# mills-lab/vapor

Hardware: AMD Instinct MI355X
Metric: SV loci validated/sec (higher is better)
Workload: dtype u32

## Files before the change

### vapor_amd/csrc/vapor_hip.hip

```cpp
#include "vapor_kernels.h"
#include "vapor_wide.h"
#include "vapor_anyk.h"
#include "vapor_realign.h"
#include "vapor_realign_trace.h"
#include "vapor_bamdev.h"
#include "vapor_bgzf.h"
#include "vapor_fasta.h"
#include "vapor_refine.h"
#include "vapor_planner.h"
#include "vapor_readplan.h"
#include "vapor_hip.h"

#include <unistd.h>

#include <algorithm>
#include <cstdio>
#include <cstdlib>
#include <cstring>
#include <new>
#include <numeric>
#include <map>
#include <memory>
#include <mutex>
#include <set>
// ... 23 lines not shown

struct BlockPool {
    std::multimap<size_t, void*> free_dev, free_host;
    std::map<const void*, size_t> cap_of;
    size_t cached_dev = 0, cached_host = 0;
};
static std::mutex g_live_m;
static std::set<const void*> g_live_ctx;

static size_t pool_round(size_t bytes)
{
    if (bytes <= 256) return 256;
    if (bytes < ((size_t)1 << 16)) { size_t c = 256; while (c < bytes) c <<= 1; return c; }
    return (bytes + 0xFFFF) & ~(size_t)0xFFFF;
}

struct vapor_ctx {
    int device = 0;
    hipStream_t stream = nullptr;
    hipStream_t own_stream = nullptr;
    hipStream_t lane[2] = {nullptr, nullptr};
    hipStream_t fin[2] = {nullptr, nullptr};
    unsigned lane_rr = 0;
    bool user_stream = false;
    uint8_t* h_stage = nullptr;
    uint8_t* d_stage = nullptr;
    size_t stage_cap = 0;
    std::vector<double> h_gt;
    double* d_gt = nullptr;
    int reads_per_task = MAX_READS_PER_TASK;
    int n_cus = 256;
    int join_tasks = 256;
    int64_t max_pair_cap = (int64_t)1 << 28;
    bool shared_join = true;
    int remap_in_clean = 1;
    int clean_order = 1;
    int clean_fit = 1;
    int64_t trace_budget = vapor_trace::BUDGET_DEFAULT;
    int stage_threads = 3;
    bool attrs_set = false;
    uint32_t* d_crc_pow = nullptr;
    std::map<const uint8_t*, size_t> arenas;
    hipStream_t bam_stream = nullptr;
    int bam_stream_share = 0;
    int bam_cu_share = 0;
    hipEvent_t bam_ev[2] = {nullptr, nullptr};
    double bam_stats[7] = {0, 0, 0, 0, 0, 0, 0};
    hipEvent_t fasta_ev[2] = {nullptr, nullptr};
    double fasta_stats[6] = {0, 0, 0, 0, 0, 0};
    BlockPool pool;
};

static bool ctx_alive(const vapor_ctx* c)
{
    std::lock_guard<std::mutex> g(g_live_m);
// ... 97 lines not shown
    int32_t n_lit = 0;
    std::vector<SeqDesc> h;
    SeqDesc* d_seqs = nullptr;
    uint32_t *d_p2 = nullptr, *d_e1 = nullptr, *d_x4 = nullptr;
    size_t plane_chunks = 0;
    std::vector<std::vector<HSeg>> derived;
    std::vector<ShareGroup> groups;
    std::vector<int32_t> group_of, slot_of;
    uint8_t* d_raw = nullptr;
    std::vector<int64_t> raw_off;
};

struct vapor_plan : PlanLayout {
    vapor_ctx* ctx = nullptr;
    int device = 0;
    vapor_seqset* set = nullptr;
    int64_t n_pairs = 0;
    std::vector<int64_t> last_stats;
    int hcap_want = 4096;
    bool hcap_measured = false;
    int64_t total_cap = 0;
    DPair* d_pairs = nullptr;
    DTask* d_tasks = nullptr;
    int32_t* d_task_pairs = nullptr;
    unsigned long long* d_hits = nullptr;
    uint8_t* d_hflags = nullptr;
    unsigned long long* d_nhits = nullptr;
    long long* d_stats = nullptr;
    long long* h_stats = nullptr;
    hipEvent_t ev[4] = {nullptr, nullptr, nullptr, nullptr};
    hipEvent_t ev_f[2] = {nullptr, nullptr};
    std::vector<std::array<hipEvent_t, 4>> ring;
    int ring_n = 0;
    bool overflow_final = false;
    double acc_ms[4] = {0, 0, 0, 0};
    int64_t acc_n = 0;
    double* h_loci = nullptr;
    hipEvent_t ev_t0 = nullptr;
    hipStream_t lane = nullptr;
    hipStream_t fin = nullptr;
    hipEvent_t ev_clean = nullptr;
    hipEvent_t ev_fin = nullptr;
    bool have_fin = false;
    hipEvent_t ev_last = nullptr;
    hipEvent_t ev_after = nullptr;
    bool have_last = false, have_after = false;
    double t_join = 0, t_clean = 0, t_total = 0;
    int n_retried = 0;
    bool ran = false;
    bool flags_valid = false;
    int64_t n_reads = 0, n_loci = 0;
    DRead* d_reads = nullptr;
    int32_t* d_locus_first = nullptr;
    double* d_gt = nullptr;
    bool own_gt = false;
    double* d_read_scores = nullptr;
    double* d_loci = nullptr;
    unsigned int* d_overflow = nullptr;
    int32_t* d_big_list = nullptr;
    unsigned int* h_overflow = nullptr;
    bool big_known = false;
    unsigned int n_big = 0;
// ... 99 lines not shown
        if (e) (void)hipEventDestroy(e);
    for (hipEvent_t e : c->fasta_ev)
        if (e) (void)hipEventDestroy(e);
    delete c;
    return VAPOR_OK;
}

extern "C" int vapor_set_param(vapor_ctx* c, const char* name, int64_t v)
{
    if (!c || !name) return fail(VAPOR_E_ARG, "vapor_set_param: null argument");
    if (!strcmp(name, "reads_per_task")) {
        if (v < 1 || v > MAX_READS_PER_TASK) return fail(VAPOR_E_ARG, "reads_per_task out of range");
        c->reads_per_task = (int)v;
        return VAPOR_OK;
    }
    if (!strcmp(name, "bam_cu_share")) {
        if (v < 0 || v > 8) return fail(VAPOR_E_ARG, "bam_cu_share out of range (0 .. 8 eighths of the CUs; 0 and 8: all)");
        c->bam_cu_share = (int)(v == 8 ? 0 : v);
        return VAPOR_OK;
    }
    if (!strcmp(name, "join_tasks")) {
        if (v < 1) return fail(VAPOR_E_ARG, "join_tasks out of range");
        c->join_tasks = (int)v;
        return VAPOR_OK;
    }
    if (!strcmp(name, "max_pair_cap")) {
        if (v < 1) return fail(VAPOR_E_ARG, "max_pair_cap out of range");
        c->max_pair_cap = v;
        return VAPOR_OK;
    }
    if (!strcmp(name, "shared_join")) {
        c->shared_join = v != 0;
        return VAPOR_OK;
    }
    if (!strcmp(name, "remap_in_clean")) {
        if (v < 0 || v > 2) return fail(VAPOR_E_ARG, "vapor_set_param: remap_in_clean is 0, 1 or 2");
        c->remap_in_clean = (int)v;
        return VAPOR_OK;
    }
    if (!strcmp(name, "clean_order")) {
        c->clean_order = v != 0 ? 1 : 0;
        return VAPOR_OK;
    }
    if (!strcmp(name, "clean_fit")) {
        c->clean_fit = v != 0;
        return VAPOR_OK;
// ... 845 lines not shown

static void plan_free_grid(vapor_plan* p)
{
    dfree(p->ctx, p->d_grid); p->d_grid = nullptr;
    dfree(p->ctx, p->d_group_out); p->d_group_out = nullptr;
    dfree(p->ctx, p->d_winner_scores); p->d_winner_scores = nullptr;
    p->n_groups = 0;
}

static void plan_free_reads(vapor_plan* p)
{
    dfree(p->ctx, p->d_reads); p->d_reads = nullptr;
    p->d_locus_first = nullptr;
    if (p->own_gt) dfree(p->ctx, p->d_gt);
    p->d_gt = nullptr; p->own_gt = false;
    dfree(p->ctx, p->d_read_scores); p->d_read_scores = nullptr;
    dfree(p->ctx, p->d_loci); p->d_loci = nullptr;
}

static void plan_free_device(vapor_plan* p)
{
    dfree(p->ctx, p->d_pairs); p->d_pairs = nullptr;
    dfree(p->ctx, p->d_tasks); p->d_tasks = nullptr;
    dfree(p->ctx, p->d_task_pairs); p->d_task_pairs = nullptr;
    dfree(p->ctx, p->d_hits); p->d_hits = nullptr;
    dfree(p->ctx, p->d_hflags); p->d_hflags = nullptr;
    dfree(p->ctx, p->d_nhits); p->d_nhits = nullptr;
    dfree(p->ctx, p->d_stats); p->d_stats = nullptr;
    plan_free_reads(p);
    dfree(p->ctx, p->d_shares); p->d_shares = nullptr;
    dfree(p->ctx, p->d_maps); p->d_maps = nullptr;
    dfree(p->ctx, p->d_serve); p->d_serve = nullptr;
    dfree(p->ctx, p->d_clean_order); p->d_clean_order = nullptr;
    plan_free_grid(p);
}

extern "C" int vapor_plan_destroy(vapor_plan* p)
{
    if (!p) return VAPOR_OK;
    (void)hipSetDevice(p->device);
    if (p->ring_n > 0 && p->lane && ctx_alive(p->ctx)) {
        (void)hipStreamSynchronize(p->lane);
        if (p->fin) (void)hipStreamSynchronize(p->fin);
    }
    plan_free_device(p);
    hfree(p->ctx, p->h_stats);
    hfree(p->ctx, p->h_overflow);
    dfree(p->ctx, p->d_overflow);
    dfree(p->ctx, p->d_big_list);
    for (auto& e : p->ev)
        if (e) (void)hipEventDestroy(e);
    for (auto& r : p->ring)
        for (auto& e : r)
            if (e) (void)hipEventDestroy(e);
    hfree(p->ctx, p->h_loci);
    for (auto& e : p->ev_f)
        if (e) (void)hipEventDestroy(e);
    if (p->ev_t0) (void)hipEventDestroy(p->ev_t0);
    if (p->ev_last) (void)hipEventDestroy(p->ev_last);
    if (p->ev_clean) (void)hipEventDestroy(p->ev_clean);
    if (p->ev_fin) (void)hipEventDestroy(p->ev_fin);
    if (p->ev_after) (void)hipEventDestroy(p->ev_after);
    delete p;
    return VAPOR_OK;
}

static_assert((2 * VAPOR_MAX_SEQ_LEN + 2 + 31) / 32 <= CLEAN_RANGE_WORDS_MAX, "cluster_axis sizes its per-thread word list for this");
// ... 15 lines not shown
    HIPCHK(hipMemcpyAsync(p->d_pairs, p->hp.data(), sizeof(DPair) * p->hp.size(), hipMemcpyHostToDevice, p->ctx->stream));
    if (p->n_dpairs) {
        for (auto& sv : p->serve)
            if (sv.dpair >= 0) { sv.hit_off = p->hp[(size_t)sv.dpair].hit_off; sv.cap = p->hp[(size_t)sv.dpair].cap; }
        HIPCHK(hipMemcpyAsync(p->d_serve, p->serve.data(), sizeof(DServe) * p->serve.size(), hipMemcpyHostToDevice, p->ctx->stream));
    }
    return VAPOR_OK;
}

extern "C" int vapor_plan_create(vapor_ctx* ctx, vapor_seqset* set, int64_t n_pairs, const vapor_pair* pairs,
                                 vapor_plan** out)
{
    if (!ctx || !set || !out || n_pairs < 0 || (n_pairs && !pairs))
        return fail(VAPOR_E_ARG, "vapor_plan_create: null argument");
    if (n_pairs > 0x7FFFFFF0LL) return fail(VAPOR_E_ARG, "too many pairs");
    HIPCHK(hipSetDevice(ctx->device));
    CallScope sc(ctx, ctx->stream);
    std::unique_ptr<vapor_plan, Building<vapor_plan, vapor_plan_destroy>> p(new (std::nothrow) vapor_plan(), {&sc});
    if (!p) return fail(VAPOR_E_NOMEM, "out of memory");
    p->ctx = ctx;
    p->device = ctx->device;
    p->set = set;
    p->n_pairs = n_pairs;
    static_cast<PlanLayout&>(*p) = plan_layout(PlanParams{ctx->reads_per_task, ctx->join_tasks, ctx->max_pair_cap, ctx->shared_join,
                                                          tile_pos<JoinCfg, 2>(), tile_pos<JoinCfg, 4>()},
                                               SetView{set->h, set->n, set->n_lit, set->derived, set->groups, set->group_of, set->slot_of},
                                               n_pairs, pairs);
    p->hcap_want = (int)std::min<int64_t>(p->hwant, CLEAN_HCAP_MAX);
    p->n_dpairs = (int64_t)p->shares.size();
    HIPCHK(dmalloc(ctx, (void**)&p->d_pairs, sizeof(DPair) * p->hp.size()));
    HIPCHK(dmalloc(ctx, (void**)&p->d_tasks, sizeof(DTask) * std::max<size_t>(p->tasks.size(), 1)));
    HIPCHK(dmalloc(ctx, (void**)&p->d_task_pairs, sizeof(int32_t) * std::max<size_t>(p->task_pairs.size(), 1)));
    HIPCHK(dmalloc(ctx, (void**)&p->d_nhits, sizeof(unsigned long long) * p->hp.size()));
    HIPCHK(hipMemsetAsync(p->d_nhits, 0, sizeof(unsigned long long) * p->hp.size(), ctx->stream));
    HIPCHK(dmalloc(ctx, (void**)&p->d_stats, sizeof(long long) * 16 * p->hp.size()));
    HIPCHK(hmalloc(ctx, (void**)&p->h_stats, sizeof(long long) * 16 * p->hp.size()));
    HIPCHK(dmalloc(ctx, (void**)&p->d_overflow, 4 * sizeof(unsigned int)));
    HIPCHK(hipMemsetAsync(p->d_overflow, 0, 4 * sizeof(unsigned int), ctx->stream));
    HIPCHK(dmalloc(ctx, (void**)&p->d_big_list, sizeof(int32_t) * p->hp.size()));
    HIPCHK(hmalloc(ctx, (void**)&p->h_overflow, 2 * sizeof(unsigned int)));
    if (p->n_dpairs) {
        HIPCHK(dmalloc(ctx, (void**)&p->d_shares, sizeof(DShare) * p->shares.size()));
        HIPCHK(dmalloc(ctx, (void**)&p->d_maps, sizeof(int32_t) * std::max<size_t>(p->tables.size(), 1)));
        HIPCHK(dmalloc(ctx, (void**)&p->d_serve, sizeof(DServe) * p->serve.size()));
        HIPCHK(hipMemcpyAsync(p->d_shares, p->shares.data(), sizeof(DShare) * p->shares.size(), hipMemcpyHostToDevice, ctx->stream));
        if (!p->tables.empty())
            HIPCHK(hipMemcpyAsync(p->d_maps, p->tables.data(), sizeof(int32_t) * p->tables.size(), hipMemcpyHostToDevice, ctx->stream));
    }
    if (ctx->clean_order && n_pairs > 1 && n_pairs <= (int64_t)8 * (2048 / CLEAN_THREADS) * ctx->n_cus) {
        HIPCHK(dmalloc(ctx, (void**)&p->d_clean_order, sizeof(int32_t) * (size_t)n_pairs));
        const std::vector<int32_t> ord = clean_order(*p, n_pairs);
        HIPCHK(hipMemcpy(p->d_clean_order, ord.data(), sizeof(int32_t) * (size_t)n_pairs, hipMemcpyHostToDevice));
    }
    for (auto& e : p->ev) HIPCHK(hipEventCreate(&e));
    for (auto& e : p->ev_f) HIPCHK(hipEventCreate(&e));
    HIPCHK(hipEventCreate(&p->ev_t0));
    if (!p->tasks.empty())
        HIPCHK(hipMemcpyAsync(p->d_tasks, p->tasks.data(), sizeof(DTask) * p->tasks.size(), hipMemcpyHostToDevice, ctx->stream));
    if (!p->task_pairs.empty())
        HIPCHK(hipMemcpyAsync(p->d_task_pairs, p->task_pairs.data(), sizeof(int32_t) * p->task_pairs.size(), hipMemcpyHostToDevice, ctx->stream));
    if (const int rc = plan_alloc_hits(p.get())) return rc;
    HIPCHK(hipStreamSynchronize(ctx->stream));
    p->last_stats.assign((size_t)n_pairs * 16, 0);
    *out = p.release();
    return VAPOR_OK;
}

template <int BPS, int K>
static void launch_join(vapor_plan* p, const Launch& L, bool first, hipStream_t st)
{
    const vapor_seqset* s = p->set;
    if (BPS == 2 && L.exc == 1)
        hipLaunchKernelGGL((join_kernel<JoinCfg, BPS, K, (BPS == 2 ? 1 : 0)>), dim3((unsigned)L.n_tasks), dim3(JoinCfg::THREADS), JOIN_DYN_LDS(BPS),
                           st, s->d_seqs, s->d_p2, s->d_e1, s->d_x4, p->d_pairs, p->d_tasks + L.task_begin,
                           p->d_task_pairs, p->d_hits, p->d_nhits, first ? p->d_overflow : (unsigned int*)nullptr);
    else if (BPS == 2 && L.exc == 2)
        hipLaunchKernelGGL((join_kernel<JoinCfg, BPS, K, (BPS == 2 ? 2 : 0)>), dim3((unsigned)L.n_tasks), dim3(JoinCfg::THREADS), JOIN_DYN_LDS(BPS),
                           st, s->d_seqs, s->d_p2, s->d_e1, s->d_x4, p->d_pairs, p->d_tasks + L.task_begin,
                           p->d_task_pairs, p->d_hits, p->d_nhits, first ? p->d_overflow : (unsigned int*)nullptr);
    else
        hipLaunchKernelGGL((join_kernel<JoinCfg, BPS, K, 0>), dim3((unsigned)L.n_tasks), dim3(JoinCfg::THREADS), JOIN_DYN_LDS(BPS),
                           st, s->d_seqs, s->d_p2, s->d_e1, s->d_x4, p->d_pairs, p->d_tasks + L.task_begin,
                           p->d_task_pairs, p->d_hits, p->d_nhits, first ? p->d_overflow : (unsigned int*)nullptr);
}

static int clean_groups_cap(int range_words_cap) { return range_words_cap * 32 / 10 + 8; }

template <typename... A>
static void launch_clean(int range_words_cap, unsigned grid, size_t lds, hipStream_t st, A... a)
{
    const int per = (range_words_cap + CLEAN_THREADS - 1) / CLEAN_THREADS;
    if (per <= 4) hipLaunchKernelGGL(clean_kernel<4>, dim3(grid), dim3(CLEAN_THREADS), lds, st, a...);
    else if (per <= 8) hipLaunchKernelGGL(clean_kernel<8>, dim3(grid), dim3(CLEAN_THREADS), lds, st, a...);
    else hipLaunchKernelGGL(clean_kernel<CLEAN_PER_MAX>, dim3(grid), dim3(CLEAN_THREADS), lds, st, a...);
}

constexpr int CLEAN_BIG_GRID = 1024;

static size_t clean_fixed_bytes(int rw, bool wide)
{
    const size_t g = (size_t)clean_groups_cap(rw);
    return sizeof(uint32_t) * ((size_t)rw + ((size_t)rw + 1) / 2 + (wide ? g : (g + 1) / 2)) + 64;
}

static int clean_groups_lds(int rw, int hcap)
// ... 23 lines not shown
        if (cap >= (exact ? want : want * 9 / 10) || per_cu == 1) { g.hcap = std::max(cap, 0); g.per_cu = per_cu; break; }
    }
    return g;
}
static CleanGeom clean_geom(int range_words_cap, int want, bool exact = false)
{
    const CleanGeom seq = clean_geom_for(range_words_cap, want, false, exact), dual = clean_geom_for(range_words_cap, want, true, exact);
#ifdef VAPOR_DEV_BUILD
    if (const char* e = getenv("VAPOR_DEV_CLEAN_DUAL")) return atoi(e) ? dual : seq;
#endif
    return dual.per_cu >= seq.per_cu ? dual : seq;
}

static int async_fold(vapor_plan* p);

static bool remap_in_clean(const vapor_plan* p)
{
    if (p->n_dpairs <= 0 || p->ctx->remap_in_clean == 0) return false;
    if (p->ctx->remap_in_clean == 2) return true;
    const CleanGeom cg = clean_geom(p->range_words_cap, p->hcap_want, p->hcap_measured);
    return p->n_pairs <= 4 * (int64_t)cg.per_cu * p->ctx->n_cus;
}

static int plan_run_once(vapor_plan* p, bool fetch_stats = true, hipEvent_t* evs = nullptr, hipStream_t on = nullptr, bool skip_big = false,
                         hipEvent_t before_clean = nullptr, bool keep_flags = true)
{
    vapor_ctx* c = p->ctx;
    hipStream_t st = on ? on : c->stream;
    hipEvent_t* ev = evs ? evs : p->ev;
    if (p->launches.empty()) HIPCHK(hipMemsetAsync(p->d_overflow, 0, 2 * sizeof(unsigned int), st));
    HIPCHK(hipEventRecord(ev[0], st));
    bool first = true;
    for (const Launch& L : p->launches) {
        if (L.bps == 2) {
            if (L.k == 10) launch_join<2, 10>(p, L, first, st);
            else if (L.k == 20) launch_join<2, 20>(p, L, first, st);
            else if (L.k == 30) launch_join<2, 30>(p, L, first, st);
            else launch_join<2, 40>(p, L, first, st);
        } else {
            if (L.k == 10) launch_join<4, 10>(p, L, first, st);
            else if (L.k == 20) launch_join<4, 20>(p, L, first, st);
            else if (L.k == 30) launch_join<4, 30>(p, L, first, st);
            else launch_join<4, 40>(p, L, first, st);
        }
        first = false;
        HIPCHK(hipGetLastError());
    }
#if defined(VAPOR_AB) && VAPOR_AB == 3
    if (false) {
#else
    if (p->n_dpairs && !remap_in_clean(p)) {
#endif
        hipLaunchKernelGGL(remap_kernel, dim3((unsigned)p->n_dpairs), dim3(256), 0, st, (const DPair*)p->d_pairs, (const DShare*)p->d_shares,
                           (const int32_t*)p->d_maps, p->d_hits, p->d_nhits, p->d_overflow);
        HIPCHK(hipGetLastError());
    }
    HIPCHK(hipEventRecord(ev[1], st));
    if (before_clean) HIPCHK(hipStreamWaitEvent(st, before_clean, 0));
    if (p->n_pairs > 0) {
        const CleanGeom cg = clean_geom(p->range_words_cap, p->hcap_want, p->hcap_measured);
        const int hcap = cg.hcap;
        size_t lds = clean_lds_bytes(p->range_words_cap, hcap, cg.dual);
#ifdef VAPOR_DEV_BUILD
        if (const char* e = getenv("VAPOR_DEV_CLEAN_PAD")) lds += (size_t)atoi(e);
#endif
        const bool in_clean = remap_in_clean(p);
// ... 15 lines not shown
    if (p->n_pairs > 0 && fetch_stats)
        HIPCHK(hipMemcpyAsync(p->h_stats, p->d_stats, sizeof(long long) * 16 * (size_t)p->n_pairs, hipMemcpyDeviceToHost, st));
    if (!fetch_stats) return VAPOR_OK;
    HIPCHK(hipEventRecord(ev[3], st));
    HIPCHK(hipStreamSynchronize(st));
    float a = 0, b = 0, t = 0;
    HIPCHK(hipEventElapsedTime(&a, ev[0], ev[1]));
    HIPCHK(hipEventElapsedTime(&b, ev[1], ev[2]));
    HIPCHK(hipEventElapsedTime(&t, ev[0], ev[3]));
    p->t_join = a; p->t_clean = b; p->t_total = t;
    return VAPOR_OK;
}

extern "C" int vapor_plan_run(vapor_plan* p, int64_t* stats)
{
    if (!p || (p->n_pairs && !stats)) return fail(VAPOR_E_ARG, "vapor_plan_run: null argument");
    HIPCHK(hipSetDevice(p->ctx->device));
    if (p->ring_n > 0) {
        int rc0 = async_fold(p);
        if (rc0 != VAPOR_OK) return rc0;
    }
    p->n_retried = 0;
    for (int attempt = 0; attempt < 3; ++attempt) {
        int rc = plan_run_once(p);
        if (rc != VAPOR_OK) return rc;
        int64_t grow = 0;
        for (int64_t i = 0; i < p->n_pairs; ++i) {
            const long long* s = p->h_stats + 16 * i;
            if (s[15] == VAPOR_E_OVERFLOW && s[14] <= p->ctx->max_pair_cap && (uint32_t)s[14] > p->hp[i].cap) {
                p->hp[i].cap = (uint32_t)s[14];
                ++grow;
            }
        }
        if (p->n_dpairs) {
            std::vector<unsigned long long> dc((size_t)p->n_dpairs);
            HIPCHK(hipMemcpy(dc.data(), p->d_nhits + p->n_pairs, sizeof(unsigned long long) * dc.size(), hipMemcpyDeviceToHost));
            for (int64_t t = 0; t < p->n_dpairs; ++t) {
                DPair& d = p->hp[(size_t)(p->n_pairs + t)];
                const uint32_t need = (uint32_t)dc[(size_t)t];
                if (need > d.cap && (int64_t)need <= p->ctx->max_pair_cap) { d.cap = need; ++grow; }
            }
        }
        if (!grow) break;
        p->n_retried += (int)grow;
        rc = plan_alloc_hits(p);
        if (rc != VAPOR_OK) return rc;
    }
// ... 14 lines not shown
        for (int64_t t = 0; t < p->n_dpairs; ++t)
            if ((uint32_t)dc[(size_t)t] > p->hp[(size_t)(p->n_pairs + t)].cap)
                for (int32_t tg : p->shares[(size_t)t].target)
                    if (tg >= 0 && p->status[(size_t)tg] == 0) p->status[(size_t)tg] = VAPOR_E_OVERFLOW;
    }
    for (int64_t i = 0; i < p->n_pairs; ++i) {
        long long* s = p->h_stats + 16 * i;
        if (p->status[i] != 0) {
            for (int t = 0; t < 16; ++t) s[t] = 0;
            s[1] = s[2] = -1;
            s[15] = p->status[i];
        }
    }
    memcpy(p->last_stats.data(), p->h_stats, sizeof(int64_t) * 16 * (size_t)p->n_pairs);
    memcpy(stats, p->h_stats, sizeof(int64_t) * 16 * (size_t)p->n_pairs);
    p->ran = true;
    return VAPOR_OK;
}

extern "C" int vapor_plan_timings(vapor_plan* p, double* ms, int32_t n)
{
    if (!p || !ms) return fail(VAPOR_E_ARG, "vapor_plan_timings: null argument");
    const CleanGeom cg = clean_geom(p->range_words_cap, p->hcap_want, p->hcap_measured);
    double v[10] = {p->t_join, p->t_clean, p->t_total, (double)p->launches.size(), (double)p->n_retried, p->t_finish,
                    (double)p->n_served, (double)p->n_dpairs, (double)cg.per_cu, remap_in_clean(p) ? 1.0 : 0.0};
    for (int i = 0; i < n && i < 10; ++i) ms[i] = v[i];
    return VAPOR_OK;
}

extern "C" int vapor_plan_record_counts(vapor_plan* p, int64_t* records)
{
    if (!p || !records) return fail(VAPOR_E_ARG, "vapor_plan_record_counts: null argument");
    if (!p->ran) return fail(VAPOR_E_ARG, "vapor_plan_record_counts: plan has not been run");
    HIPCHK(hipSetDevice(p->ctx->device));
    std::vector<unsigned long long> cnt((size_t)std::max<int64_t>(p->n_pairs, 1));
    HIPCHK(hipMemcpy(cnt.data(), p->d_nhits, sizeof(unsigned long long) * (size_t)p->n_pairs, hipMemcpyDeviceToHost));
    for (int64_t i = 0; i < p->n_pairs; ++i) records[i] = (int64_t)(uint32_t)cnt[i];
    return VAPOR_OK;
}

extern "C" int vapor_plan_algorithmic_bytes(vapor_plan* p, int64_t* bytes, int64_t* cells)
{
    if (!p || !bytes || !cells) return fail(VAPOR_E_ARG, "null argument");
    int64_t b = 0, c = 0;
    for (int64_t i = 0; i < p->n_pairs; ++i) {
        if (p->status[i] != 0) continue;
        int64_t n1 = p->set->h[p->hp[i].seq1].len;
        int64_t n2 = std::max<int64_t>(0, (int64_t)p->set->h[p->hp[i].seq2].len - p->hp[i].off2);
        int64_t nh = p->ran ? p->last_stats[16 * i] : 0;
// ... 787 lines not shown
extern "C" int vapor_plan_run_loci(vapor_plan* p, void* d_loci_out, double* loci_out, double* read_scores)
{
    if (!p) return fail(VAPOR_E_ARG, "vapor_plan_run_loci: null plan");
    if (!p->d_reads) return fail(VAPOR_E_ARG, "vapor_plan_run_loci: call vapor_plan_set_reads first");
    HIPCHK(hipSetDevice(p->ctx->device));
    if (p->ring_n > 0) {
        int rc0 = async_fold(p);
        if (rc0 != VAPOR_OK) return rc0;
    }
    hipStream_t st = p->ctx->stream;
    bool host_status = false;
    for (int64_t i = 0; i < p->n_pairs; ++i)
        if (p->status[i] != 0) { host_status = true; break; }
    int rc;
    const bool light = !(host_status || !p->ran);
    if (!light) {
        rc = vapor_plan_run(p, p->last_stats.data());
        if (rc != VAPOR_OK) return rc;
        for (int64_t i = 0; i < p->n_pairs && !host_status; ++i)
            if (p->status[i] != 0) host_status = true;
        if (host_status)
            HIPCHK(hipMemcpyAsync(p->d_stats, p->h_stats, sizeof(long long) * 16 * (size_t)p->n_pairs, hipMemcpyHostToDevice, st));
    } else {
        rc = plan_run_once(p, false, nullptr, nullptr, false, nullptr, false);
        if (rc != VAPOR_OK) return rc;
    }
    hipEvent_t e1 = p->ev_f[1];
    double* d_out = d_loci_out ? static_cast<double*>(d_loci_out) : p->d_loci;
    if (p->n_loci > 0) {
        hipLaunchKernelGGL(finish_kernel, dim3((unsigned)p->n_loci), dim3(64), 0, st, p->d_reads, p->d_locus_first, p->d_stats,
                           p->d_gt, p->d_read_scores, d_out, (double*)nullptr);
        HIPCHK(hipGetLastError());
    }
    HIPCHK(hipEventRecord(e1, st));
    if (p->n_groups > 0 && p->n_loci > 0) {
        const size_t ng = (size_t)p->n_groups;
        int32_t* d_idx = p->d_grid + 2 * ng + 2;
        hipLaunchKernelGGL(grid_pick_kernel, dim3((unsigned)ng), dim3(64), 0, st, d_out, p->d_grid, p->d_locus_first, p->d_read_scores,
                           p->d_grid + ng + 1, d_idx, p->d_group_out, p->d_winner_scores);
        HIPCHK(hipGetLastError());
        if (p->grid_idx_out) HIPCHK(hipMemcpyAsync(p->grid_idx_out, d_idx, sizeof(int32_t) * ng, hipMemcpyDeviceToHost, st));
        if (p->grid_rec_out) HIPCHK(hipMemcpyAsync(p->grid_rec_out, p->d_group_out, sizeof(double) * 16 * ng, hipMemcpyDeviceToHost, st));
        if (p->grid_scores_out && p->n_grid_scores)
            HIPCHK(hipMemcpyAsync(p->grid_scores_out, p->d_winner_scores, sizeof(double) * (size_t)p->n_grid_scores, hipMemcpyDeviceToHost, st));
    }
    HIPCHK(hipMemcpyAsync(p->h_overflow, p->d_overflow, 2 * sizeof(unsigned int), hipMemcpyDeviceToHost, st));
    if (loci_out && p->n_loci)
// ... 131 lines not shown
    if (!c) return fail(VAPOR_E_ARG, "vapor_set_stream: null context");
    c->stream = hip_stream ? static_cast<hipStream_t>(hip_stream) : c->own_stream;
    c->user_stream = hip_stream != nullptr;
    return VAPOR_OK;
}

static int plan_lane(vapor_plan* p, hipStream_t* out)
{
    vapor_ctx* c = p->ctx;
    if (c->user_stream) { *out = c->stream; return VAPOR_OK; }
    if (!p->lane) {
        const unsigned l = c->lane_rr++ & 1u;
        if (!c->lane[l]) HIPCHK(hipStreamCreateWithFlags(&c->lane[l], hipStreamNonBlocking));
        if (!c->fin[l]) {
            int lo = 0, hi = 0;
            if (hipDeviceGetStreamPriorityRange(&lo, &hi) != hipSuccess ||
                hipStreamCreateWithPriority(&c->fin[l], hipStreamNonBlocking, hi) != hipSuccess) {
                (void)hipGetLastError();
                c->fin[l] = nullptr;
                HIPCHK(hipStreamCreateWithFlags(&c->fin[l], hipStreamNonBlocking));
            }
        }
        p->lane = c->lane[l];
        p->fin = c->fin[l];
    }
    *out = p->lane;
    return VAPOR_OK;
}

static int async_fold(vapor_plan* p)
{
    hipStream_t st = nullptr;
    int rc = plan_lane(p, &st);
    if (rc != VAPOR_OK) return rc;
    if (p->lane && p->lane != st) HIPCHK(hipStreamSynchronize(p->lane));
    HIPCHK(hipStreamSynchronize(st));
    if (p->fin && p->fin != st) HIPCHK(hipStreamSynchronize(p->fin));
    for (int i = 0; i < p->ring_n; ++i) {
        float x = 0;
        hipEvent_t* ev = p->ring[(size_t)i].data();
        HIPCHK(hipEventElapsedTime(&x, ev[0], ev[1])); p->acc_ms[0] += x;
        HIPCHK(hipEventElapsedTime(&x, ev[1], ev[2])); p->acc_ms[1] += x;
        HIPCHK(hipEventElapsedTime(&x, ev[2], ev[3])); p->acc_ms[2] += x;
        HIPCHK(hipEventElapsedTime(&x, ev[0], ev[3])); p->acc_ms[3] += x;
    }
    p->acc_n += p->ring_n;
// ... 12 lines not shown
    if (p->ring_n >= ASYNC_RING) {
        int rc0 = async_fold(p);
        if (rc0 != VAPOR_OK) return rc0;
    }
    hipStream_t st = nullptr;
    int rc = plan_lane(p, &st);
    if (rc != VAPOR_OK) return rc;
    if (p->ring.empty()) {
        p->ring.resize(ASYNC_RING);
        for (auto& r : p->ring)
            for (auto& e : r) { e = nullptr; HIPCHK(hipEventCreate(&e)); }
        HIPCHK(hmalloc(p->ctx, (void**)&p->h_loci, sizeof(double) * 8 * (size_t)std::max<int64_t>(p->n_loci, 1)));
        HIPCHK(hipEventCreateWithFlags(&p->ev_last, hipEventDisableTiming));
        HIPCHK(hipEventCreateWithFlags(&p->ev_clean, hipEventDisableTiming));
        HIPCHK(hipEventCreateWithFlags(&p->ev_fin, hipEventDisableTiming));
    }
    hipStream_t fs = (p->fin && !p->ctx->user_stream) ? p->fin : st;
    if (p->have_after) {
        HIPCHK(hipStreamWaitEvent(fs, p->ev_after, 0));
        p->have_after = false;
    }
    if (p->ring_n == 0 && p->acc_n == 0) HIPCHK(hipMemsetAsync(p->d_overflow + 2, 0, sizeof(unsigned int), st));
    hipEvent_t* ev = p->ring[(size_t)p->ring_n].data();
    rc = plan_run_once(p, false, ev, st, p->big_known && p->n_big == 0, (fs != st && p->have_fin) ? p->ev_fin : nullptr, false);
    if (rc != VAPOR_OK) return rc;
    double* d_out = d_loci_out ? static_cast<double*>(d_loci_out) : p->d_loci;
    if (fs != st) {
        HIPCHK(hipEventRecord(p->ev_clean, st));
        HIPCHK(hipStreamWaitEvent(fs, p->ev_clean, 0));
    }
    if (p->n_loci > 0) {
        hipLaunchKernelGGL(finish_kernel, dim3((unsigned)p->n_loci), dim3(64), 0, fs, p->d_reads, p->d_locus_first, p->d_stats,
                           p->d_gt, p->d_read_scores, d_out, p->h_loci);
        HIPCHK(hipGetLastError());
    }
    HIPCHK(hipEventRecord(ev[3], fs));
    HIPCHK(hipEventRecord(p->ev_last, fs));
    if (fs != st) {
        HIPCHK(hipEventRecord(p->ev_fin, fs));
        p->have_fin = true;
    }
    p->have_last = true;
    ++p->ring_n;
    return VAPOR_OK;
}

extern "C" int vapor_plan_then(vapor_plan* p, void* hip_stream)
{
    if (!p) return fail(VAPOR_E_ARG, "vapor_plan_then: null plan");
    if (!p->have_last) return VAPOR_OK;
    HIPCHK(hipSetDevice(p->ctx->device));
    HIPCHK(hipStreamWaitEvent(static_cast<hipStream_t>(hip_stream), p->ev_last, 0));
    return VAPOR_OK;
}

extern "C" int vapor_plan_after(vapor_plan* p, void* hip_stream)
{
    if (!p) return fail(VAPOR_E_ARG, "vapor_plan_after: null plan");
    HIPCHK(hipSetDevice(p->ctx->device));
    if (!p->ev_after) HIPCHK(hipEventCreateWithFlags(&p->ev_after, hipEventDisableTiming));
    HIPCHK(hipEventRecord(p->ev_after, static_cast<hipStream_t>(hip_stream)));
    p->have_after = true;
    return VAPOR_OK;
}

// ... 68 lines not shown
```

### vapor_amd/csrc/vapor_planner.h

```cpp
#pragma once
#include "vapor_records.h"
#include "vapor_hip.h"

#include <algorithm>
#include <cstring>
#include <map>
#include <utility>
#include <vector>

#ifndef VAPOR_BUILD_COST_X8
#define VAPOR_BUILD_COST_X8 6
#endif

namespace vapor {

struct HSeg { int32_t parent, off, len, dst; bool rc; };
struct SharePiece {
    int32_t slot;
    int32_t a_from, a_to;
    int32_t tile_off;
};
struct ShareGroup {
    int32_t parent = -1;
    bool upper = false;
// ... 72 lines not shown
                t_len += a1 - a0;
            };
            for (auto& r : mapped) {
                if (r.first > u) add_piece(u, r.first - 1);
                u = std::max(u, r.second + 1);
            }
            if (u <= n_a - 1) add_piece(u, n_a - 1);
        }
        if (t_len > VAPOR_MAX_SEQ_LEN || t_len > (int64_t)2 * n_r + 4096) { g.members.clear(); g.pieces.clear(); continue; }
        g.t_seq = n + (int32_t)hidden.size();
        hidden.push_back(std::move(t));
        if (g.identity >= 0) { (*group_of)[(size_t)g.identity] = (int32_t)q; (*slot_of)[(size_t)g.identity] = 0; }
        for (size_t m = 0; m < g.members.size(); ++m) { (*group_of)[(size_t)g.members[m]] = (int32_t)q; (*slot_of)[(size_t)g.members[m]] = (int32_t)m + 1; }
    }
    return hidden;
}

struct PlanParams {
    int reads_per_task;
    int join_tasks;
    int64_t max_pair_cap;
    bool shared_join;
    int tile2, tile4;
};
struct SetView {
    const std::vector<SeqDesc>& h;
    int32_t n, n_lit;
    const std::vector<std::vector<HSeg>>& derived;
    const std::vector<ShareGroup>& groups;
    const std::vector<int32_t>& group_of;
    const std::vector<int32_t>& slot_of;
};

struct PlanLayout {
    std::vector<DPair> hp;
    std::vector<int32_t> status;
    std::vector<DTask> tasks;
    std::vector<int32_t> task_pairs;
    std::vector<Launch> launches;
    std::vector<DShare> shares;
    std::vector<int32_t> tables;
    std::vector<DServe> serve;
    int64_t n_served = 0;
    int range_words_cap = 1;
    int64_t hwant = 1024;
};

inline int pair_mode(const SeqDesc& s1, const SeqDesc& s2)
{
    return (s1.n_exc > 0 && s2.n_exc > 0) ? 4 : (s2.n_exc > 0 ? 3 : (s1.n_exc > 0 ? 5 : 2));
}
inline Launch launch_of_mode(int m, int k, int task_begin) { return Launch{m == 4 ? 4 : 2, k, task_begin, 0, m == 3 ? 1 : m == 5 ? 2 : 0}; }

inline uint32_t pair_slot_cap(int64_t n1, int64_t n2, int64_t max_pair_cap)
{
    return (uint32_t)std::min<int64_t>(std::min(n1, n2) + ((n1 * n2) >> 17) + 1024, max_pair_cap);
}

inline int allele_tiles(const PlanParams& P, int32_t len_a, int k, int m)
{
    const int ta = m != 4 ? P.tile2 : P.tile4;
    return std::max(1, (len_a - k + 1 + ta - 1) / ta);
// ... 148 lines not shown
        for (int t = 0; t < 4; ++t) {
            sh.target[t] = tgt[t];
            if (tgt[t] >= 0) {
                served[(size_t)tgt[t]] = 1; ++L->n_served;
                DServe& sv = L->serve[(size_t)tgt[t]];
                sv.dpair = sh.dpair; sv.iv_first = sh.iv_first; sv.n_iv = sh.n_iv; sv.slot = t;
                sv.pad = counted ? 0 : 1;
                counted = true;
            }
        }
        L->hp.push_back(d);
        mode->push_back((uint8_t)md);
        L->shares.push_back(sh);
    }
    if (!L->shares.empty()) {
        std::vector<int32_t> kept;
        kept.reserve(order->size());
        for (int32_t x : *order) if (!served[(size_t)x]) kept.push_back(x);
        for (size_t t = 0; t < L->shares.size(); ++t) kept.push_back((int32_t)(n_pairs + (int64_t)t));
        order->swap(kept);
    }
}

inline void plan_launch_tasks(const PlanParams& P, const SetView& S, size_t q, size_t e, int m, PlanLayout* L)
{
    const std::vector<int32_t>& order = L->task_pairs;
    const int k = L->hp[order[q]].k;
    const size_t n = e - q;
    std::vector<int64_t> probe(n), build(n);
    int64_t total = 0, biggest = 0;
    for (size_t t = q; t < e; ++t) {
        const DPair& d = L->hp[order[t]];
        probe[t - q] = (int64_t)S.h[d.seq1].len * allele_tiles(P, S.h[d.seq2].len, k, m) + 256;
        build[t - q] = (VAPOR_BUILD_COST_X8 * (int64_t)S.h[d.seq2].len) / 8;
        total += probe[t - q] + build[t - q];
        biggest = std::max(biggest, probe[t - q] + build[t - q]);
    }
    int64_t want = std::max<int64_t>(1, std::min<int64_t>((int64_t)n, P.join_tasks));
    {
        const int64_t need = ((int64_t)n + P.reads_per_task - 1) / P.reads_per_task;
        if (need > want) want = std::min<int64_t>((int64_t)n, (need + want - 1) / want * want);
    }
    std::vector<int64_t> inside(n);
    for (size_t t = 0; t < n; ++t)
        inside[t] = probe[t] + ((t > 0 && L->hp[order[q + t]].seq2 != L->hp[order[q + t - 1]].seq2) ? build[t] : 0);
    auto pack = [&](int64_t bound, std::vector<size_t>* cuts) {
        int64_t ranges = 0, acc = 0;
        size_t t0 = 0;
        for (size_t t = 0; t < n; ++t) {
            const int64_t add = t == t0 ? probe[t] + build[t] : inside[t];
            const bool full = (int)(t - t0) >= P.reads_per_task;
            if (t > t0 && (acc + add > bound || full)) {
                ++ranges;
                if (cuts) cuts->push_back(t0);
                t0 = t;
                acc = probe[t] + build[t];
            } else {
// ... 4 lines not shown
        if (cuts) cuts->push_back(t0);
        return ranges;
    };
    int64_t in_sum = 0;
    for (size_t t = 0; t < n; ++t) in_sum += inside[t];
    int64_t lo = std::max(biggest, in_sum / want), hi = lo;
    while (hi < total && pack(hi, nullptr) > want) { lo = hi + 1; hi = std::min(total, hi * 2); }
    while (lo < hi) {
        const int64_t mid = lo + (hi - lo) / 2;
        if (pack(mid, nullptr) <= want) hi = mid; else lo = mid + 1;
    }
    std::vector<size_t> cuts;
    pack(lo, &cuts);
    L->launches.push_back(launch_of_mode(m, k, (int)L->tasks.size()));
    for (size_t c = 0; c < cuts.size(); ++c) {
        const size_t t0 = q + cuts[c], t1 = q + (c + 1 < cuts.size() ? cuts[c + 1] : n);
        DTask tk;
        tk.seq2 = L->hp[order[t0]].seq2; tk.k = k; tk.n_reads = (int32_t)(t1 - t0); tk.first = (int32_t)t0;
        L->tasks.push_back(tk);
        L->launches.back().n_tasks++;
    }
}

inline PlanLayout plan_layout(const PlanParams& P, const SetView& S, int64_t n_pairs, const vapor_pair* pairs)
{
    PlanLayout L;
    std::vector<int32_t> order;
    std::vector<uint8_t> mode;
    plan_pairs(P, S, n_pairs, pairs, &L, &mode, &order);
    if (P.shared_join && !S.groups.empty() && n_pairs > 0) plan_shared_joins(P, S, n_pairs, &L, &mode, &order);
    {
        std::vector<std::pair<uint64_t, int32_t>> keyed(order.size());
        for (size_t t = 0; t < order.size(); ++t) {
            const int32_t x = order[t];
            keyed[t] = {((uint64_t)mode[(size_t)x] << 48) | ((uint64_t)(uint32_t)L.hp[(size_t)x].k << 32) | (uint32_t)L.hp[(size_t)x].seq2, x};
        }
        std::sort(keyed.begin(), keyed.end());
        for (size_t t = 0; t < order.size(); ++t) order[t] = keyed[t].second;
    }
    L.task_pairs = std::move(order);
    const std::vector<int32_t>& tp = L.task_pairs;
    for (size_t q = 0; q < tp.size();) {
        size_t e = q;
        const int m = mode[tp[q]], k = L.hp[tp[q]].k;
        while (e < tp.size() && mode[tp[e]] == m && L.hp[tp[e]].k == k) ++e;
        plan_launch_tasks(P, S, q, e, m, &L);
        q = e;
    }
    return L;
}

inline int64_t clean_cost(const PlanLayout& L, int64_t i)
{
    const DPair& d = L.hp[(size_t)i];
    const bool c1 = d.flags & VAPOR_PF_C1, c2 = d.flags & VAPOR_PF_C2, dir = (d.flags & VAPOR_PF_DIR) && c1;
    int64_t w = 4 + (c1 ? 8 : 0) + (c2 ? (c1 ? 5 : 8) : 0) + (dir ? 7 : 0);
    if (!L.serve.empty() && L.serve[(size_t)i].dpair >= 0) w += L.serve[(size_t)i].slot == 0 ? 2 : 4;
    const int64_t size = std::min<int64_t>(d.len1, std::max(0, d.len2 - d.off2));
    return L.status[(size_t)i] == 0 ? w * size : 0;
}
inline std::vector<int32_t> clean_order(const PlanLayout& L, int64_t n_pairs)
{
    std::vector<std::pair<int64_t, int32_t>> cost((size_t)n_pairs);
    for (int64_t i = 0; i < n_pairs; ++i) cost[(size_t)i] = {-clean_cost(L, i), (int32_t)i};
    std::stable_sort(cost.begin(), cost.end());
    std::vector<int32_t> ord((size_t)n_pairs);
    for (int64_t i = 0; i < n_pairs; ++i) ord[(size_t)i] = cost[(size_t)i].second;
    return ord;
}

}
// ... 1 lines not shown
```

### vapor_amd/engine.py

```python
from __future__ import annotations

import ctypes
import weakref
from typing import Iterable, List, Optional, Sequence, Tuple

import numpy as np

from . import _lib as L


_utf8 = ctypes.pythonapi.PyUnicode_AsUTF8AndSize
_utf8.restype = ctypes.c_void_p
_utf8.argtypes = [ctypes.py_object, ctypes.POINTER(ctypes.c_ssize_t)]


def _ascii_data_offset() -> int:
    probe = "ACGTACGTACGTACGT" * 4
    size = ctypes.c_ssize_t()
    p = _utf8(probe, ctypes.byref(size))
    return (p - id(probe)) if p and size.value == len(probe) else -1


_ASCII_OFF = _ascii_data_offset()

# ... 200 lines not shown
            self.close()
        except Exception:
            pass


class Plan:
    def __init__(self, engine: "Engine", seqset: SeqSet, pairs: np.ndarray):
        self.engine = engine
        self.seqset = seqset
        self.pairs = np.ascontiguousarray(pairs, dtype=L.PAIR_DTYPE)
        self.n = len(self.pairs)
        h = ctypes.c_void_p()
        L.check(L.load().vapor_plan_create(engine._ctx, seqset._h, self.n, self.pairs.ctypes.data_as(ctypes.c_void_p),
                                           ctypes.byref(h)))
        self._h = h
        engine._live.add(self)
        self.stats = np.zeros((max(self.n, 1), L.STATS_STRIDE), dtype=np.int64)

    def run(self) -> np.ndarray:
        L.check(L.load().vapor_plan_run(self._h, L.ptr(self.stats, ctypes.c_int64)))
        return self.stats[:self.n]

    def timings(self) -> dict:
        ms = np.zeros(10, dtype=np.float64)
        L.check(L.load().vapor_plan_timings(self._h, L.ptr(ms, ctypes.c_double), 10))
        return {"join_ms": ms[0], "clean_ms": ms[1], "total_ms": ms[2], "join_launches": int(ms[3]),
                "retried_pairs": int(ms[4]), "finish_ms": ms[5], "pairs_served_by_shared_joins": int(ms[6]), "shared_joins": int(ms[7]),
                "clean_workgroups_per_cu": int(ms[8]), "remap_in_clean": int(ms[9])}

    def record_counts(self) -> np.ndarray:
        out = np.zeros(max(self.n, 1), dtype=np.int64)
        L.check(L.load().vapor_plan_record_counts(self._h, L.ptr(out, ctypes.c_int64)))
        return out[:self.n]

    def set_reads(self, reads: np.ndarray, n_loci: int) -> None:
        from . import finish
        self.reads = np.ascontiguousarray(reads, dtype=L.READ_DTYPE)
        self.n_loci = int(n_loci)
        L.check(L.load().vapor_plan_set_reads(self._h, len(self.reads), self.reads.ctypes.data_as(ctypes.c_void_p),
                                              self.n_loci, L.ptr(finish.gt_table(), ctypes.c_double)))
        self.loci = np.zeros((max(self.n_loci, 1), L.LOCUS_STRIDE), dtype=np.float64)
        self.read_scores = np.zeros(max(len(self.reads), 1), dtype=np.float64)

    def run_loci(self, device_out: int = 0, want_host: bool = True, want_scores: bool = False):
        L.check(L.load().vapor_plan_run_loci(self._h, ctypes.c_void_p(device_out) if device_out else None,
                                             L.ptr(self.loci, ctypes.c_double) if want_host else None,
                                             L.ptr(self.read_scores, ctypes.c_double) if want_scores else None))
        return self.loci[:self.n_loci]

    def set_grid(self, first_locus: np.ndarray) -> None:
        fn = Engine._wide_entry("vapor_plan_set_grid", "refinement kernel")
# ... 368 lines not shown
```

Before: 804,500.

## Add allele-aligned join task table used when another lane's plan overlaps

```diff
diff --git a/vapor_amd/csrc/vapor_hip.hip b/vapor_amd/csrc/vapor_hip.hip
--- a/vapor_amd/csrc/vapor_hip.hip
+++ b/vapor_amd/csrc/vapor_hip.hip
@@ -69,6 +69,7 @@
     hipStream_t lane[2] = {nullptr, nullptr};
     hipStream_t fin[2] = {nullptr, nullptr};
     unsigned lane_rr = 0;
+    vapor_plan* lane_plan[2] = {nullptr, nullptr};
     bool user_stream = false;
     uint8_t* h_stage = nullptr;
     uint8_t* d_stage = nullptr;
@@ -78,6 +79,7 @@
     int reads_per_task = MAX_READS_PER_TASK;
     int n_cus = 256;
     int join_tasks = 256;
+    int join_align = 1;
     int64_t max_pair_cap = (int64_t)1 << 28;
     bool shared_join = true;
     int remap_in_clean = 1;
@@ -221,6 +223,11 @@
     int64_t total_cap = 0;
     DPair* d_pairs = nullptr;
     DTask* d_tasks = nullptr;
+    DTask* d_atasks = nullptr;
+    int join_align = 0;
+    PlanParams params{};
+    bool aligned_made = false;
+    int last_table = 0;
     int32_t* d_task_pairs = nullptr;
     unsigned long long* d_hits = nullptr;
     uint8_t* d_hflags = nullptr;
@@ -237,6 +244,7 @@
     double* h_loci = nullptr;
     hipEvent_t ev_t0 = nullptr;
     hipStream_t lane = nullptr;
+    int lane_ix = -1;
     hipStream_t fin = nullptr;
     hipEvent_t ev_clean = nullptr;
     hipEvent_t ev_fin = nullptr;
@@ -382,6 +390,11 @@
     if (!strcmp(name, "join_tasks")) {
         if (v < 1) return fail(VAPOR_E_ARG, "join_tasks out of range");
         c->join_tasks = (int)v;
+        return VAPOR_OK;
+    }
+    if (!strcmp(name, "join_align")) {
+        if (v < 0 || v > 2) return fail(VAPOR_E_ARG, "vapor_set_param: join_align is 0, 1 or 2");
+        c->join_align = (int)v;
         return VAPOR_OK;
     }
     if (!strcmp(name, "max_pair_cap")) {
@@ -1273,6 +1286,7 @@
 {
     dfree(p->ctx, p->d_pairs); p->d_pairs = nullptr;
     dfree(p->ctx, p->d_tasks); p->d_tasks = nullptr;
+    dfree(p->ctx, p->d_atasks); p->d_atasks = nullptr;
     dfree(p->ctx, p->d_task_pairs); p->d_task_pairs = nullptr;
     dfree(p->ctx, p->d_hits); p->d_hits = nullptr;
     dfree(p->ctx, p->d_hflags); p->d_hflags = nullptr;
@@ -1294,6 +1308,9 @@
         (void)hipStreamSynchronize(p->lane);
         if (p->fin) (void)hipStreamSynchronize(p->fin);
     }
+    if (ctx_alive(p->ctx))
+        for (auto& q : p->ctx->lane_plan)
+            if (q == p) q = nullptr;
     plan_free_device(p);
     hfree(p->ctx, p->h_stats);
     hfree(p->ctx, p->h_overflow);
@@ -1355,10 +1372,13 @@
     p->device = ctx->device;
     p->set = set;
     p->n_pairs = n_pairs;
-    static_cast<PlanLayout&>(*p) = plan_layout(PlanParams{ctx->reads_per_task, ctx->join_tasks, ctx->max_pair_cap, ctx->shared_join,
-                                                          tile_pos<JoinCfg, 2>(), tile_pos<JoinCfg, 4>()},
+    p->params = PlanParams{ctx->reads_per_task, ctx->join_tasks, ctx->max_pair_cap, ctx->shared_join,
+                           tile_pos<JoinCfg, 2>(), tile_pos<JoinCfg, 4>(), ctx->join_align == 2};
+    static_cast<PlanLayout&>(*p) = plan_layout(p->params,
                                                SetView{set->h, set->n, set->n_lit, set->derived, set->groups, set->group_of, set->slot_of},
                                                n_pairs, pairs);
+    p->join_align = ctx->join_align;
+    if (p->join_align == 2) { p->tasks = p->atasks; p->launches = p->alaunches; p->model[0] = p->model[1]; }
     p->hcap_want = (int)std::min<int64_t>(p->hwant, CLEAN_HCAP_MAX);
     p->n_dpairs = (int64_t)p->shares.size();
     HIPCHK(dmalloc(ctx, (void**)&p->d_pairs, sizeof(DPair) * p->hp.size()));
@@ -1400,20 +1420,20 @@
 }
 
 template <int BPS, int K>
-static void launch_join(vapor_plan* p, const Launch& L, bool first, hipStream_t st)
+static void launch_join(vapor_plan* p, const Launch& L, const DTask* d_tasks, bool first, hipStream_t st)
 {
     const vapor_seqset* s = p->set;
     if (BPS == 2 && L.exc == 1)
         hipLaunchKernelGGL((join_kernel<JoinCfg, BPS, K, (BPS == 2 ? 1 : 0)>), dim3((unsigned)L.n_tasks), dim3(JoinCfg::THREADS), JOIN_DYN_LDS(BPS),
-                           st, s->d_seqs, s->d_p2, s->d_e1, s->d_x4, p->d_pairs, p->d_tasks + L.task_begin,
+                           st, s->d_seqs, s->d_p2, s->d_e1, s->d_x4, p->d_pairs, d_tasks + L.task_begin,
                            p->d_task_pairs, p->d_hits, p->d_nhits, first ? p->d_overflow : (unsigned int*)nullptr);
     else if (BPS == 2 && L.exc == 2)
         hipLaunchKernelGGL((join_kernel<JoinCfg, BPS, K, (BPS == 2 ? 2 : 0)>), dim3((unsigned)L.n_tasks), dim3(JoinCfg::THREADS), JOIN_DYN_LDS(BPS),
-                           st, s->d_seqs, s->d_p2, s->d_e1, s->d_x4, p->d_pairs, p->d_tasks + L.task_begin,
+                           st, s->d_seqs, s->d_p2, s->d_e1, s->d_x4, p->d_pairs, d_tasks + L.task_begin,
                            p->d_task_pairs, p->d_hits, p->d_nhits, first ? p->d_overflow : (unsigned int*)nullptr);
     else
         hipLaunchKernelGGL((join_kernel<JoinCfg, BPS, K, 0>), dim3((unsigned)L.n_tasks), dim3(JoinCfg::THREADS), JOIN_DYN_LDS(BPS),
-                           st, s->d_seqs, s->d_p2, s->d_e1, s->d_x4, p->d_pairs, p->d_tasks + L.task_begin,
+                           st, s->d_seqs, s->d_p2, s->d_e1, s->d_x4, p->d_pairs, d_tasks + L.task_begin,
                            p->d_task_pairs, p->d_hits, p->d_nhits, first ? p->d_overflow : (unsigned int*)nullptr);
 }
 
@@ -1483,26 +1503,57 @@
     return p->n_pairs <= 4 * (int64_t)cg.per_cu * p->ctx->n_cus;
 }
 
-static int plan_run_once(vapor_plan* p, bool fetch_stats = true, hipEvent_t* evs = nullptr, hipStream_t on = nullptr, bool skip_big = false,
+constexpr int JOIN_ALIGN_MIN_SAVING_PM = 15;
+constexpr int JOIN_ALIGN_MAX_DEARER_PCT = 10;
+static bool join_align_pays(const TableModel& bal, const TableModel& ali)
+{
+    return ali.n_tasks > 0 && (bal.sum - ali.sum) * 1000 >= bal.sum * JOIN_ALIGN_MIN_SAVING_PM && ali.path * 100 <= bal.path * (100 + JOIN_ALIGN_MAX_DEARER_PCT);
+}
+static int join_table_for_async(vapor_plan* p, hipStream_t st, int* table)
+{
+    *table = 0;
+    if (p->join_align != 1) return VAPOR_OK;
+    const vapor_ctx* c = p->ctx;
+    if (c->user_stream || p->lane_ix < 0) return VAPOR_OK;
+    const vapor_plan* o = c->lane_plan[1 - p->lane_ix];
+    if (!o || o == p || o->ring_n <= 0) return VAPOR_OK;
+    if (!p->aligned_made) {
+        const vapor_seqset* s = p->set;
+        plan_aligned(p->params, SetView{s->h, s->n, s->n_lit, s->derived, s->groups, s->group_of, s->slot_of}, p);
+        p->aligned_made = true;
+        if (!p->atasks.empty() && join_align_pays(p->model[0], p->model[1])) {
+            HIPCHK(dmalloc(p->ctx, (void**)&p->d_atasks, sizeof(DTask) * p->atasks.size()));
+            HIPCHK(hipMemcpyAsync(p->d_atasks, p->atasks.data(), sizeof(DTask) * p->atasks.size(), hipMemcpyHostToDevice, st));
+        }
+    }
+    if (p->d_atasks) *table = 1;
+    return VAPOR_OK;
+}
+
+static int plan_run_once(vapor_plan* p, int table, bool fetch_stats = true, hipEvent_t* evs = nullptr, hipStream_t on = nullptr, bool skip_big = false,
                          hipEvent_t before_clean = nullptr, bool keep_flags = true)
 {
     vapor_ctx* c = p->ctx;
     hipStream_t st = on ? on : c->stream;
     hipEvent_t* ev = evs ? evs : p->ev;
-    if (p->launches.empty()) HIPCHK(hipMemsetAsync(p->d_overflow, 0, 2 * sizeof(unsigned int), st));
+    if (table == 1 && !p->d_atasks) table = 0;
+    const std::vector<Launch>& launches = table == 1 ? p->alaunches : p->launches;
+    const DTask* d_tasks = table == 1 ? p->d_atasks : p->d_tasks;
+    p->last_table = table;
+    if (launches.empty()) HIPCHK(hipMemsetAsync(p->d_overflow, 0, 2 * sizeof(unsigned int), st));
     HIPCHK(hipEventRecord(ev[0], st));
     bool first = true;
-    for (const Launch& L : p->launches) {
+    for (const Launch& L : launches) {
         if (L.bps == 2) {
-            if (L.k == 10) launch_join<2, 10>(p, L, first, st);
-            else if (L.k == 20) launch_join<2, 20>(p, L, first, st);
-            else if (L.k == 30) launch_join<2, 30>(p, L, first, st);
-            else launch_join<2, 40>(p, L, first, st);
+            if (L.k == 10) launch_join<2, 10>(p, L, d_tasks, first, st);
+            else if (L.k == 20) launch_join<2, 20>(p, L, d_tasks, first, st);
+            else if (L.k == 30) launch_join<2, 30>(p, L, d_tasks, first, st);
+            else launch_join<2, 40>(p, L, d_tasks, first, st);
         } else {
-            if (L.k == 10) launch_join<4, 10>(p, L, first, st);
-            else if (L.k == 20) launch_join<4, 20>(p, L, first, st);
-            else if (L.k == 30) launch_join<4, 30>(p, L, first, st);
-            else launch_join<4, 40>(p, L, first, st);
+            if (L.k == 10) launch_join<4, 10>(p, L, d_tasks, first, st);
+            else if (L.k == 20) launch_join<4, 20>(p, L, d_tasks, first, st);
+            else if (L.k == 30) launch_join<4, 30>(p, L, d_tasks, first, st);
+            else launch_join<4, 40>(p, L, d_tasks, first, st);
         }
         first = false;
         HIPCHK(hipGetLastError());
@@ -1564,7 +1615,7 @@
     }
     p->n_retried = 0;
     for (int attempt = 0; attempt < 3; ++attempt) {
-        int rc = plan_run_once(p);
+        int rc = plan_run_once(p, 0);
         if (rc != VAPOR_OK) return rc;
         int64_t grow = 0;
         for (int64_t i = 0; i < p->n_pairs; ++i) {
@@ -1625,9 +1676,11 @@
 {
     if (!p || !ms) return fail(VAPOR_E_ARG, "vapor_plan_timings: null argument");
     const CleanGeom cg = clean_geom(p->range_words_cap, p->hcap_want, p->hcap_measured);
-    double v[10] = {p->t_join, p->t_clean, p->t_total, (double)p->launches.size(), (double)p->n_retried, p->t_finish,
-                    (double)p->n_served, (double)p->n_dpairs, (double)cg.per_cu, remap_in_clean(p) ? 1.0 : 0.0};
-    for (int i = 0; i < n && i < 10; ++i) ms[i] = v[i];
+    const TableModel& tm = p->model[p->last_table];
+    double v[12] = {p->t_join, p->t_clean, p->t_total, (double)p->launches.size(), (double)p->n_retried, p->t_finish,
+                    (double)p->n_served, (double)p->n_dpairs, (double)cg.per_cu, remap_in_clean(p) ? 1.0 : 0.0,
+                    (double)tm.n_tasks, (double)tm.builds};
+    for (int i = 0; i < n && i < 12; ++i) ms[i] = v[i];
     return VAPOR_OK;
 }
 
@@ -2461,7 +2514,7 @@
         if (host_status)
             HIPCHK(hipMemcpyAsync(p->d_stats, p->h_stats, sizeof(long long) * 16 * (size_t)p->n_pairs, hipMemcpyHostToDevice, st));
     } else {
-        rc = plan_run_once(p, false, nullptr, nullptr, false, nullptr, false);
+        rc = plan_run_once(p, 0, false, nullptr, nullptr, false, nullptr, false);
         if (rc != VAPOR_OK) return rc;
     }
     hipEvent_t e1 = p->ev_f[1];
@@ -2639,6 +2692,7 @@
             }
         }
         p->lane = c->lane[l];
+        p->lane_ix = (int)l;
         p->fin = c->fin[l];
     }
     *out = p->lane;
@@ -2697,7 +2751,10 @@
     }
     if (p->ring_n == 0 && p->acc_n == 0) HIPCHK(hipMemsetAsync(p->d_overflow + 2, 0, sizeof(unsigned int), st));
     hipEvent_t* ev = p->ring[(size_t)p->ring_n].data();
-    rc = plan_run_once(p, false, ev, st, p->big_known && p->n_big == 0, (fs != st && p->have_fin) ? p->ev_fin : nullptr, false);
+    int table = 0;
+    rc = join_table_for_async(p, st, &table);
+    if (rc != VAPOR_OK) return rc;
+    rc = plan_run_once(p, table, false, ev, st, p->big_known && p->n_big == 0, (fs != st && p->have_fin) ? p->ev_fin : nullptr, false);
     if (rc != VAPOR_OK) return rc;
     double* d_out = d_loci_out ? static_cast<double*>(d_loci_out) : p->d_loci;
     if (fs != st) {
@@ -2716,6 +2773,7 @@
         p->have_fin = true;
     }
     p->have_last = true;
+    if (!p->ctx->user_stream && p->lane_ix >= 0) p->ctx->lane_plan[p->lane_ix] = p;
     ++p->ring_n;
     return VAPOR_OK;
 }
diff --git a/vapor_amd/csrc/vapor_planner.h b/vapor_amd/csrc/vapor_planner.h
--- a/vapor_amd/csrc/vapor_planner.h
+++ b/vapor_amd/csrc/vapor_planner.h
@@ -118,6 +118,7 @@
     int64_t max_pair_cap;
     bool shared_join;
     int tile2, tile4;
+    bool align_tasks = false;
 };
 struct SetView {
     const std::vector<SeqDesc>& h;
@@ -128,12 +129,17 @@
     const std::vector<int32_t>& slot_of;
 };
 
+struct TableModel { int64_t sum = 0, path = 0, builds = 0, n_tasks = 0; };
+
 struct PlanLayout {
     std::vector<DPair> hp;
     std::vector<int32_t> status;
     std::vector<DTask> tasks;
     std::vector<int32_t> task_pairs;
     std::vector<Launch> launches;
+    std::vector<DTask> atasks;
+    std::vector<Launch> alaunches;
+    TableModel model[2];
     std::vector<DShare> shares;
     std::vector<int32_t> tables;
     std::vector<DServe> serve;
@@ -328,6 +334,12 @@
     }
 }
 
+inline int64_t probe_cost(const PlanParams& P, const SetView& S, const DPair& d, int k, int m)
+{
+    return (int64_t)S.h[d.seq1].len * allele_tiles(P, S.h[d.seq2].len, k, m) + 256;
+}
+inline int64_t build_cost(const SetView& S, const DPair& d) { return (VAPOR_BUILD_COST_X8 * (int64_t)S.h[d.seq2].len) / 8; }
+
 inline void plan_launch_tasks(const PlanParams& P, const SetView& S, size_t q, size_t e, int m, PlanLayout* L)
 {
     const std::vector<int32_t>& order = L->task_pairs;
@@ -337,8 +349,8 @@
     int64_t total = 0, biggest = 0;
     for (size_t t = q; t < e; ++t) {
         const DPair& d = L->hp[order[t]];
-        probe[t - q] = (int64_t)S.h[d.seq1].len * allele_tiles(P, S.h[d.seq2].len, k, m) + 256;
-        build[t - q] = (VAPOR_BUILD_COST_X8 * (int64_t)S.h[d.seq2].len) / 8;
+        probe[t - q] = probe_cost(P, S, d, k, m);
+        build[t - q] = build_cost(S, d);
         total += probe[t - q] + build[t - q];
         biggest = std::max(biggest, probe[t - q] + build[t - q]);
     }
@@ -389,6 +401,116 @@
     }
 }
 
+inline void plan_launch_aligned(const PlanParams& P, const SetView& S, size_t q, size_t e, int m, PlanLayout* L)
+{
+    const std::vector<int32_t>& order = L->task_pairs;
+    const int k = L->hp[order[q]].k;
+    const size_t n = e - q;
+    std::vector<int64_t> probe(n);
+    std::vector<size_t> group{0};
+    int64_t total = 0, biggest = 0;
+    for (size_t t = 0; t < n; ++t) {
+        const DPair& d = L->hp[order[q + t]];
+        probe[t] = probe_cost(P, S, d, k, m);
+        if (t > 0 && d.seq2 != L->hp[order[q + t - 1]].seq2) group.push_back(t);
+        total += probe[t] + build_cost(S, d);
+        biggest = std::max(biggest, probe[t] + build_cost(S, d));
+    }
+    group.push_back(n);
+    const size_t n_g = group.size() - 1;
+    auto pack = [&](size_t g, int64_t bound, std::vector<size_t>* cuts) {
+        const int64_t build = build_cost(S, L->hp[order[q + group[g]]]);
+        int64_t ranges = 0, acc = 0;
+        size_t t0 = group[g];
+        for (size_t t = group[g]; t < group[g + 1]; ++t) {
+            if (t > t0 && (acc + probe[t] > bound || (int)(t - t0) >= P.reads_per_task)) {
+                ++ranges;
+                if (cuts) cuts->push_back(t0);
+                t0 = t;
+                acc = 0;
+            }
+            if (t == t0) acc = build;
+            acc += probe[t];
+        }
+        if (cuts) cuts->push_back(t0);
+        return ranges + 1;
+    };
+    auto pack_all = [&](int64_t bound) {
+        int64_t ranges = 0;
+        for (size_t g = 0; g < n_g; ++g) ranges += pack(g, bound, nullptr);
+        return ranges;
+    };
+    const int64_t want = std::max(1, P.join_tasks);
+    int64_t lo = biggest, hi = total;
+    if (pack_all(hi) <= want)
+        while (lo < hi) {
+            const int64_t mid = lo + (hi - lo) / 2;
+            if (pack_all(mid) <= want) hi = mid; else lo = mid + 1;
+        }
+    const int64_t bound = hi;
+    L->alaunches.push_back(launch_of_mode(m, k, (int)L->atasks.size()));
+    std::vector<size_t> cuts;
+    for (size_t g = 0; g < n_g; ++g) {
+        const int64_t m_g = pack(g, bound, nullptr);
+        int64_t glo = 0, ghi = bound;
+        for (size_t t = group[g]; t < group[g + 1]; ++t) glo = std::max(glo, probe[t]);
+        glo += build_cost(S, L->hp[order[q + group[g]]]);
+        while (glo < ghi) {
+            const int64_t mid = glo + (ghi - glo) / 2;
+            if (pack(g, mid, nullptr) <= m_g) ghi = mid; else glo = mid + 1;
+        }
+        cuts.clear();
+        pack(g, ghi, &cuts);
+        for (size_t c = 0; c < cuts.size(); ++c) {
+            const size_t t0 = q + cuts[c], t1 = q + (c + 1 < cuts.size() ? cuts[c + 1] : group[g + 1]);
+            DTask tk;
+            tk.seq2 = L->hp[order[t0]].seq2; tk.k = k; tk.n_reads = (int32_t)(t1 - t0); tk.first = (int32_t)t0;
+            L->atasks.push_back(tk);
+            L->alaunches.back().n_tasks++;
+        }
+    }
+}
+
+inline int mode_of_launch(const Launch& la) { return la.bps == 4 ? 4 : (la.exc == 1 ? 3 : la.exc == 2 ? 5 : 2); }
+
+inline TableModel table_model(const PlanParams& P, const SetView& S, const PlanLayout& L, const std::vector<DTask>& tasks,
+                              const std::vector<Launch>& launches)
+{
+    TableModel M;
+    for (const Launch& la : launches) {
+        const int m = mode_of_launch(la);
+        int64_t dearest = 0;
+        for (int x = 0; x < la.n_tasks; ++x) {
+            const DTask& tk = tasks[(size_t)(la.task_begin + x)];
+            int64_t cost = 0;
+            for (int32_t t = tk.first; t < tk.first + tk.n_reads; ++t) {
+                const DPair& d = L.hp[(size_t)L.task_pairs[(size_t)t]];
+                cost += probe_cost(P, S, d, la.k, m);
+                if (t == tk.first || d.seq2 != L.hp[(size_t)L.task_pairs[(size_t)t - 1]].seq2) {
+                    cost += build_cost(S, d);
+                    M.builds += allele_tiles(P, S.h[d.seq2].len, la.k, m);
+                }
+            }
+            M.sum += cost;
+            dearest = std::max(dearest, cost);
+        }
+        M.path += dearest;
+        M.n_tasks += la.n_tasks;
+    }
+    return M;
+}
+
+inline void plan_aligned(const PlanParams& P, const SetView& S, PlanLayout* L)
+{
+    L->atasks.clear();
+    L->alaunches.clear();
+    for (const Launch& la : L->launches) {
+        const DTask &t0 = L->tasks[(size_t)la.task_begin], &t1 = L->tasks[(size_t)(la.task_begin + la.n_tasks - 1)];
+        plan_launch_aligned(P, S, (size_t)t0.first, (size_t)(t1.first + t1.n_reads), mode_of_launch(la), L);
+    }
+    L->model[1] = table_model(P, S, *L, L->atasks, L->alaunches);
+}
+
 inline PlanLayout plan_layout(const PlanParams& P, const SetView& S, int64_t n_pairs, const vapor_pair* pairs)
 {
     PlanLayout L;
@@ -414,6 +536,8 @@
         plan_launch_tasks(P, S, q, e, m, &L);
         q = e;
     }
+    L.model[0] = table_model(P, S, L, L.tasks, L.launches);
+    if (P.align_tasks) plan_aligned(P, S, &L);
     return L;
 }
 
diff --git a/vapor_amd/engine.py b/vapor_amd/engine.py
--- a/vapor_amd/engine.py
+++ b/vapor_amd/engine.py
@@ -246,11 +246,12 @@
         return self.stats[:self.n]
 
     def timings(self) -> dict:
-        ms = np.zeros(10, dtype=np.float64)
-        L.check(L.load().vapor_plan_timings(self._h, L.ptr(ms, ctypes.c_double), 10))
+        ms = np.zeros(12, dtype=np.float64)
+        L.check(L.load().vapor_plan_timings(self._h, L.ptr(ms, ctypes.c_double), 12))
         return {"join_ms": ms[0], "clean_ms": ms[1], "total_ms": ms[2], "join_launches": int(ms[3]),
                 "retried_pairs": int(ms[4]), "finish_ms": ms[5], "pairs_served_by_shared_joins": int(ms[6]), "shared_joins": int(ms[7]),
-                "clean_workgroups_per_cu": int(ms[8]), "remap_in_clean": int(ms[9])}
+                "clean_workgroups_per_cu": int(ms[8]), "remap_in_clean": int(ms[9]),
+                "join_tasks": int(ms[10]), "table_builds": int(ms[11])}
 
     def record_counts(self) -> np.ndarray:
         out = np.zeros(max(self.n, 1), dtype=np.int64)
```

Measured after the change: 821,400 (median of 6 runs). 2.1% higher.
